# paulmillr/noble-curves

Measured on NVIDIA H100. Metric: BLS12-381 G1 MSM points/sec at 2^20 scalars, higher is better.
Workload: dtype u32-limb integer (381-bit Fp, Montgomery)

## Files before the change

### noble-curves_b200/csrc/ec.cuh

```cuda
#pragma once
#include "curve_consts.cuh"
#include "field.cuh"
#include "inv_divsteps.cuh"
#include "fp2.cuh"

namespace nmsm {

#if defined(__CUDACC__)
template <class F, bool FULLWARP>
struct Par4 {
  static constexpr int WORDS = sizeof(F) / 4;
  __device__ static __forceinline__ F bcast(const F& z, int src) {
    F r;
    const uint32_t* s = reinterpret_cast<const uint32_t*>(&z);
    uint32_t* d = reinterpret_cast<uint32_t*>(&r);
    const unsigned qbase = FULLWARP ? 0u : (threadIdx.x & 28u);
    const unsigned qmask = FULLWARP ? 0xffffffffu : (0xFu << qbase);
#pragma unroll
    for (int k = 0; k < WORDS; k++) d[k] = __shfl_sync(qmask, s[k], qbase + src);
    return r;
  }
  __device__ static __forceinline__ F pick(int l, const F& a0, const F& a1, const F& a2, const F& a3) {
    F r;
    const uint32_t* p0 = reinterpret_cast<const uint32_t*>(&a0);
// ... 3 lines not shown
    uint32_t* d = reinterpret_cast<uint32_t*>(&r);
    const uint32_t m0 = 0u - (uint32_t)(l == 0), m1 = 0u - (uint32_t)(l == 1), m2 = 0u - (uint32_t)(l == 2),
                   m3 = 0u - (uint32_t)(l == 3);
#pragma unroll
    for (int k = 0; k < WORDS; k++) d[k] = (p0[k] & m0) | (p1[k] & m1) | (p2[k] & m2) | (p3[k] & m3);
    return r;
  }
  __device__ static __forceinline__ void mul4(F& r0, F& r1, F& r2, F& r3, const F& a0, const F& b0, const F& a1,
                                              const F& b1, const F& a2, const F& b2, const F& a3, const F& b3) {
    const int l = threadIdx.x & 3;
    F x = pick(l, a0, a1, a2, a3), y = pick(l, b0, b1, b2, b3);
    F z = x * y;
    r0 = bcast(z, 0);
    r1 = bcast(z, 1);
    r2 = bcast(z, 2);
    r3 = bcast(z, 3);
  }
};
#endif

template <class F>
struct SwXyzz {
  using Field = F;
  static constexpr int COORD_WORDS = F::LIMBS;
  static constexpr int IN_WORDS = 2 * F::LIMBS;
  static constexpr int AFF_WORDS = 2 * F::LIMBS;
  static constexpr int ACC_WORDS = 4 * F::LIMBS;
  static constexpr int COST_MADD = 10, COST_ADD = 14, COST_DBL = 9;
  static constexpr bool IS_EDWARDS = false;

  struct Affine {
    F x, y;
  };
  struct Acc {
    F X, Y, ZZ, ZZZ;
  };

  NMSM_HD static Acc identity() { return Acc{F::zero(), F::one(), F::zero(), F::zero()}; }
  NMSM_HD static bool is_identity(const Acc& p) { return p.ZZ.is_zero(); }
  NMSM_HD static bool affine_is_identity(const Affine& a) { return a.x.is_zero() && a.y.is_zero(); }
  NMSM_HD static Affine prepare(const uint32_t* xy) {
    return Affine{F::from_canonical(xy), F::from_canonical(xy + F::LIMBS)};
  }
  NMSM_HD static bool input_in_range(const uint32_t* xy) {
    return F::canonical_in_range(xy) && F::canonical_in_range(xy + F::LIMBS);
  }
  NMSM_HD static Affine neg(const Affine& a) { return Affine{a.x, -a.y}; }
  NMSM_HD static Affine cneg(const Affine& a, bool n) {
    F ny = -a.y;
    return Affine{a.x, n ? ny : a.y};
  }
  NMSM_HD static Acc from_affine(const Affine& a) {
    if (affine_is_identity(a)) return identity();
    return Acc{a.x, a.y, F::one(), F::one()};
  }
  NMSM_HD static Acc neg(const Acc& p) { return Acc{p.X, -p.Y, p.ZZ, p.ZZZ}; }

  NMSM_HD static Acc dbl_affine(const Affine& a) {
    F U = nmsm::dbl(a.y);
    F V = sqr(U);
    F W = U * V;
    F S = a.x * V;
    F xx = sqr(a.x);
    F M = nmsm::dbl(xx) + xx;
    F X3 = sqr(M) - nmsm::dbl(S);
    F Y3 = M * (S - X3) - W * a.y;
    return Acc{X3, Y3, V, W};
  }
  NMSM_HD static void dbl(Acc& p) {
    if (is_identity(p)) return;
    F U = nmsm::dbl(p.Y);
    F V = sqr(U);
    F W = U * V;
    F S = p.X * V;
    F xx = sqr(p.X);
    F M = nmsm::dbl(xx) + xx;
    F X3 = sqr(M) - nmsm::dbl(S);
    F Y3 = M * (S - X3) - W * p.Y;
    p.ZZ = V * p.ZZ;
    p.ZZZ = W * p.ZZZ;
    p.X = X3;
    p.Y = Y3;
  }
  NMSM_HD static void madd(Acc& p, const Affine& a) {
    if (affine_is_identity(a)) return;
    if (is_identity(p)) {
      p = Acc{a.x, a.y, F::one(), F::one()};
      return;
    }
    F U2 = a.x * p.ZZ;
    F S2 = a.y * p.ZZZ;
    F P = U2 - p.X;
    F R = S2 - p.Y;
    if (P.is_zero()) {
      if (R.is_zero())
        p = dbl_affine(a);
      else
        p = identity();
      return;
    }
    F PP = sqr(P);
    F PPP = P * PP;
    F Q = p.X * PP;
    F X3 = sqr(R) - PPP - nmsm::dbl(Q);
    F Y3 = R * (Q - X3) - p.Y * PPP;
    p.ZZ = p.ZZ * PP;
    p.ZZZ = p.ZZZ * PPP;
    p.X = X3;
    p.Y = Y3;
  }
  NMSM_HD static void add(Acc& p, const Acc& q) {
    if (is_identity(q)) return;
    if (is_identity(p)) {
      p = q;
      return;
    }
    F U1 = p.X * q.ZZ;
    F U2 = q.X * p.ZZ;
    F S1 = p.Y * q.ZZZ;
    F S2 = q.Y * p.ZZZ;
    F P = U2 - U1;
    F R = S2 - S1;
    if (P.is_zero()) {
      if (R.is_zero())
        dbl(p);
      else
        p = identity();
      return;
    }
    F PP = sqr(P);
    F PPP = P * PP;
    F Q = U1 * PP;
    F X3 = sqr(R) - PPP - nmsm::dbl(Q);
    F Y3 = R * (Q - X3) - S1 * PPP;
    p.ZZ = p.ZZ * q.ZZ * PP;
    p.ZZZ = p.ZZZ * q.ZZZ * PPP;
    p.X = X3;
    p.Y = Y3;
  }
#if defined(__CUDACC__)
  template <bool FW>
  __device__ static void par_dbl(Acc& p) {
    if (is_identity(p)) return;
    using P4 = Par4<F, FW>;
    F U = nmsm::dbl(p.Y);
    F V, A, t2, t3;
    P4::mul4(V, A, t2, t3, U, U, p.X, p.X, U, U, U, U);
    F M = nmsm::dbl(A) + A;
    F W, S, MM;
    P4::mul4(W, S, MM, t3, U, V, p.X, V, M, M, M, M);
    F X3 = MM - nmsm::dbl(S);
    F y0, y1, zz, zzz;
    P4::mul4(y0, y1, zz, zzz, M, S - X3, W, p.Y, V, p.ZZ, W, p.ZZZ);
    p.X = X3;
    p.Y = y0 - y1;
    p.ZZ = zz;
    p.ZZZ = zzz;
  }
  template <bool FW>
  __device__ static void par_add(Acc& p, const Acc& q) {
    if (is_identity(q)) return;
    if (is_identity(p)) {
      p = q;
      return;
    }
    using P4 = Par4<F, FW>;
    F U1, U2, S1, S2;
    P4::mul4(U1, U2, S1, S2, p.X, q.ZZ, q.X, p.ZZ, p.Y, q.ZZZ, q.Y, p.ZZZ);
    F P = U2 - U1;
    F R = S2 - S1;
    if (P.is_zero()) {
      if (R.is_zero())
        par_dbl<FW>(p);
      else
        p = identity();
      return;
    }
    F PP, RR, ZZ12, ZZZ12;
    P4::mul4(PP, RR, ZZ12, ZZZ12, P, P, R, R, p.ZZ, q.ZZ, p.ZZZ, q.ZZZ);
    F PPP, Q, ZZ3, t3;
    P4::mul4(PPP, Q, ZZ3, t3, P, PP, U1, PP, ZZ12, PP, P, PP);
    F X3 = RR - PPP - nmsm::dbl(Q);
    F y0, y1, ZZZ3;
    P4::mul4(y0, y1, ZZZ3, t3, R, Q - X3, S1, PPP, ZZZ12, PPP, R, R);
    p.X = X3;
    p.Y = y0 - y1;
    p.ZZ = ZZ3;
    p.ZZZ = ZZZ3;
  }
#endif
// ... 240 lines not shown
```

### noble-curves_b200/csrc/field.cuh

```cuda
#pragma once
#include "bigint.cuh"

namespace nmsm {

template <class C>
NMSM_HD void reduce_once(uint32_t* r, uint32_t top) {
  constexpr int N = C::N;
  uint32_t d[N];
  d[0] = sub_cc(r[0], C::P(0));
#pragma unroll
  for (int k = 1; k < N; k++) d[k] = subc_cc(r[k], C::P(k));
  uint32_t t = subc(top, 0);
  bool keep = (t >> 31) != 0;
#pragma unroll
  for (int k = 0; k < N; k++) r[k] = keep ? r[k] : d[k];
}

template <class C>
NMSM_HD void mont_mul(uint32_t* r, const uint32_t* a, const uint32_t* b) {
  constexpr int N = C::N;
  static_assert(N % 2 == 0, "even limb count expected");
  uint32_t E[2 * N + 2], O[2 * N + 2];
#pragma unroll
  for (int k = 0; k < 2 * N + 2; k++) {
// ... 247 lines not shown
  NMSM_HD friend Fp operator*(const Fp& a, const Fp& b) {
#if defined(__CUDA_ARCH__) && defined(NMSM_MUL_NOINLINE)
    return mul_call<C>(a, b);
#else
    Fp r;
    mont_mul<C>(r.v, a.v, b.v);
    return r;
#endif
  }
  NMSM_HD friend Fp operator+(const Fp& a, const Fp& b) {
    Fp r;
    r.v[0] = add_cc(a.v[0], b.v[0]);
#pragma unroll
    for (int k = 1; k < N; k++) r.v[k] = addc_cc(a.v[k], b.v[k]);
    uint32_t top = addc(0, 0);
    reduce_once<C>(r.v, top);
    return r;
  }
  NMSM_HD friend Fp operator-(const Fp& a, const Fp& b) {
    Fp r;
    r.v[0] = sub_cc(a.v[0], b.v[0]);
#pragma unroll
    for (int k = 1; k < N; k++) r.v[k] = subc_cc(a.v[k], b.v[k]);
    uint32_t mask = subc(0, 0);
    r.v[0] = add_cc(r.v[0], C::P(0) & mask);
#pragma unroll
    for (int k = 1; k < N; k++) r.v[k] = addc_cc(r.v[k], C::P(k) & mask);
    return r;
  }
  NMSM_HD Fp operator-() const { return zero() - *this; }

  NMSM_HD static Fp from_canonical(const uint32_t* x) {
    Fp a, r2;
#pragma unroll
    for (int k = 0; k < N; k++) {
      a.v[k] = x[k];
      r2.v[k] = C::R2(k);
    }
    return a * r2;
  }
  NMSM_HD void to_canonical(uint32_t* x) const {
    Fp o;
#pragma unroll
    for (int k = 0; k < N; k++) o.v[k] = (k == 0) ? 1u : 0u;
    Fp r = (*this) * o;
#pragma unroll
    for (int k = 0; k < N; k++) x[k] = r.v[k];
  }
  NMSM_HD static bool canonical_in_range(const uint32_t* x) {
    uint32_t t = sub_cc(x[0], C::P(0));
#pragma unroll
    for (int k = 1; k < N; k++) t = subc_cc(x[k], C::P(k));
    (void)t;
    return subc(0, 0) != 0;
  }
};

#if defined(__CUDACC__)
template <class C>
__device__ __noinline__ Fp<C> mul_call(Fp<C> a, Fp<C> b) {
  Fp<C> r;
  mont_mul<C>(r.v, a.v, b.v);
  return r;
}
template <class C>
__device__ __noinline__ Fp<C> sqr_call(Fp<C> a) {
  Fp<C> r;
  mont_sqr<C>(r.v, a.v);
  return r;
}
#endif

template <class C>
NMSM_HD Fp<C> sqr(const Fp<C>& a) {
#if defined(__CUDA_ARCH__) && defined(NMSM_MUL_NOINLINE)
  return sqr_call<C>(a);
#else
  Fp<C> r;
  mont_sqr<C>(r.v, a.v);
  return r;
#endif
}
template <class C>
NMSM_HD Fp<C> dbl(const Fp<C>& a) {
  return a + a;
}

template <class C>
NMSM_HD Fp<C> inv_xgcd(const Fp<C>& a) {
  constexpr int N = C::N;
  if (a.is_zero()) return a;
  uint32_t u[N], v[N], x1[N], x2[N];
#pragma unroll
  for (int k = 0; k < N; k++) {
    u[k] = a.v[k];
    v[k] = C::P(k);
    x1[k] = (k == 0) ? 1u : 0u;
    x2[k] = 0u;
  }
  auto is_one = [](const uint32_t* x) {
    uint32_t t = x[0] ^ 1u;
#pragma unroll
    for (int k = 1; k < N; k++) t |= x[k];
    return t == 0;
  };
  auto halve = [](uint32_t* x, uint32_t top) {
#pragma unroll
    for (int k = 0; k < N - 1; k++) x[k] = (x[k] >> 1) | (x[k + 1] << 31);
    x[N - 1] = (x[N - 1] >> 1) | (top << 31);
  };
  auto halve_mod = [&](uint32_t* x) {
    uint32_t top = 0;
    if (x[0] & 1u) {
      x[0] = add_cc(x[0], C::P(0));
#pragma unroll
      for (int k = 1; k < N; k++) x[k] = addc_cc(x[k], C::P(k));
      top = addc(0, 0);
    }
    halve(x, top);
  };
  auto geq = [](const uint32_t* x, const uint32_t* y) {
    uint32_t t = sub_cc(x[0], y[0]);
#pragma unroll
    for (int k = 1; k < N; k++) t = subc_cc(x[k], y[k]);
    (void)t;
    return subc(0, 0) == 0;
  };
  auto sub_plain = [](uint32_t* x, const uint32_t* y) {
    x[0] = sub_cc(x[0], y[0]);
#pragma unroll
    for (int k = 1; k < N; k++) x[k] = subc_cc(x[k], y[k]);
  };
  auto sub_mod = [](uint32_t* x, const uint32_t* y) {
    x[0] = sub_cc(x[0], y[0]);
#pragma unroll
    for (int k = 1; k < N; k++) x[k] = subc_cc(x[k], y[k]);
    uint32_t mask = subc(0, 0);
    x[0] = add_cc(x[0], C::P(0) & mask);
#pragma unroll
    for (int k = 1; k < N; k++) x[k] = addc_cc(x[k], C::P(k) & mask);
  };
  while (!is_one(u) && !is_one(v)) {
    while (!(u[0] & 1u)) {
      halve(u, 0);
      halve_mod(x1);
    }
    while (!(v[0] & 1u)) {
      halve(v, 0);
      halve_mod(x2);
    }
    if (geq(u, v)) {
      sub_plain(u, v);
      sub_mod(x1, x2);
    } else {
      sub_plain(v, u);
      sub_mod(x2, x1);
    }
  }
  Fp<C> r, r2;
  const bool pick_u = is_one(u);
#pragma unroll
  for (int k = 0; k < N; k++) {
    r.v[k] = pick_u ? x1[k] : x2[k];
    r2.v[k] = C::R2(k);
  }
  return (r * r2) * r2;
// ... 4 lines not shown
```

### noble-curves_b200/csrc/msm.cuh

```cuda
#pragma once
#include <cuda_runtime.h>
#include <stdint.h>

#include "msm_body.cuh"
#include "validate.cuh"

namespace nmsm {

template <class Cv>
__global__ void k_prepare(const uint32_t* __restrict__ pts, uint32_t n, uint32_t* __restrict__ aff,
                          unsigned int* err) {
  uint32_t i = blockIdx.x * blockDim.x + threadIdx.x;
  if (i < n) prepare_body<Cv>(i, n, pts, aff, err);
}

template <class Cv, bool SCATTER>
__global__ void k_digits(const uint32_t* __restrict__ scalars, uint32_t n, MsmPlan plan,
                         unsigned int* __restrict__ counts_or_cursor, uint32_t* __restrict__ sorted,
                         unsigned int* err) {
  uint32_t i = blockIdx.x * blockDim.x + threadIdx.x;
  if (i < n) digits_body<Cv, SCATTER>(i, n, scalars, plan, counts_or_cursor, sorted, err);
}

static constexpr int SCAN_THREADS = 256;
// ... 10 lines not shown
  return t;
}

static __global__ void __launch_bounds__(SCAN_THREADS)
k_scan_tiles(const unsigned int* __restrict__ counts, uint32_t G, uint32_t* __restrict__ tile_sums) {
  __shared__ uint32_t sh[SCAN_THREADS / 32];
  const uint32_t base = blockIdx.x * SCAN_TILE + threadIdx.x * SCAN_PER_THREAD;
  uint32_t v = 0;
#pragma unroll
  for (int k = 0; k < SCAN_PER_THREAD; k++)
    if (base + k < G) v += counts[base + k];
  uint32_t t = block_sum_256(v, sh);
  if (threadIdx.x == 0) tile_sums[blockIdx.x] = t;
}

static __global__ void __launch_bounds__(SCAN_THREADS)
k_scan_apply(const unsigned int* __restrict__ counts, uint32_t G, const uint32_t* __restrict__ tile_sums,
             uint32_t* __restrict__ offsets, unsigned int* __restrict__ cursor) {
  __shared__ uint32_t sh[SCAN_THREADS / 32];
  __shared__ uint32_t warp_tot[SCAN_THREADS / 32];
  uint32_t pre = 0;
  for (uint32_t k = threadIdx.x; k < blockIdx.x; k += SCAN_THREADS) pre += tile_sums[k];
  const uint32_t tile_prefix = block_sum_256(pre, sh);
  const uint32_t base = blockIdx.x * SCAN_TILE + threadIdx.x * SCAN_PER_THREAD;
  uint32_t c[SCAN_PER_THREAD];
  uint32_t mine = 0;
#pragma unroll
  for (int k = 0; k < SCAN_PER_THREAD; k++) {
    c[k] = (base + k < G) ? counts[base + k] : 0;
    mine += c[k];
  }
  const uint32_t lane = threadIdx.x & 31, warp = threadIdx.x >> 5;
  uint32_t inc = mine;
  for (int d = 1; d < 32; d <<= 1) {
    uint32_t o = __shfl_up_sync(0xffffffffu, inc, d);
    if (lane >= (uint32_t)d) inc += o;
  }
  if (lane == 31) warp_tot[warp] = inc;
  __syncthreads();
  uint32_t wpre = 0;
  for (uint32_t q = 0; q < warp; q++) wpre += warp_tot[q];
  uint32_t run = tile_prefix + wpre + inc - mine;
#pragma unroll
  for (int k = 0; k < SCAN_PER_THREAD; k++) {
    if (base + k < G) {
      offsets[base + k] = run;
      cursor[base + k] = run;
    }
    run += c[k];
  }
  if (base < G && base + SCAN_PER_THREAD >= G) offsets[G] = run;
}

template <class F>
__device__ __forceinline__ F shfl_field(const F& a, int src_lane) {
  F r;
  const uint32_t* s = reinterpret_cast<const uint32_t*>(&a);
  uint32_t* d = reinterpret_cast<uint32_t*>(&r);
#pragma unroll
  for (int k = 0; k < (int)(sizeof(F) / 4); k++) d[k] = __shfl_sync(0xffffffffu, s[k], src_lane);
  return r;
}
template <class F>
__device__ __noinline__ F warp_batch_inverse(const F& z) {
  const int lane = threadIdx.x & 31;
  F pre = z, suf = z;
  for (int d = 1; d < 32; d <<= 1) {
    F a = shfl_field(pre, lane >= d ? lane - d : lane);
    F b = shfl_field(suf, lane + d < 32 ? lane + d : lane);
    if (lane >= d) pre = pre * a;
    if (lane + d < 32) suf = suf * b;
  }
  F r = inv(shfl_field(pre, 31));
  F left = shfl_field(pre, lane > 0 ? lane - 1 : 0);
  F right = shfl_field(suf, lane < 31 ? lane + 1 : 31);
  if (lane > 0) r = r * left;
  if (lane < 31) r = r * right;
  return r;
}

#ifndef NMSM_PAIRED
#define NMSM_PAIRED 0
#endif
#ifndef NMSM_ACC_MINBLOCKS_WIDE
#define NMSM_ACC_MINBLOCKS_WIDE 2
#endif
#ifndef NMSM_ACC_WIDE_BYTES
#define NMSM_ACC_WIDE_BYTES 257
#endif
#ifndef NMSM_ACC_MINBLOCKS
#define NMSM_ACC_MINBLOCKS 4
#endif
template <class Cv>
__global__ void __launch_bounds__(128, (sizeof(typename Cv::G::Acc) >= NMSM_ACC_WIDE_BYTES ? NMSM_ACC_MINBLOCKS_WIDE : NMSM_ACC_MINBLOCKS))
k_accumulate(const uint32_t* __restrict__ aff, const uint32_t* __restrict__ sorted,
             const uint32_t* __restrict__ offsets, MsmPlan plan, uint32_t w0, uint32_t* __restrict__ buckets,
             uint32_t* __restrict__ heads, uint32_t* __restrict__ tails) {
  const uint32_t gid = blockIdx.x * blockDim.x + threadIdx.x;
  const uint32_t w = w0 + gid / plan.TPW, t = gid % plan.TPW;
#if NMSM_PAIRED
  if constexpr (!Cv::G::IS_EDWARDS) {
    using F = typename Cv::G::Field;
    F suf[MAX_PAIRS];
    int npairs;
    const F run = accumulate_pairs_pass1<Cv>(w, t, aff, sorted, offsets, plan, suf, npairs);
    const F inv_all = warp_batch_inverse(run);
    accumulate_pairs_pass2<Cv>(w, t, aff, sorted, offsets, plan, suf, npairs, inv_all, buckets, heads, tails);
    return;
  }
#endif
  accumulate_body<Cv>(w, t, aff, sorted, offsets, plan, buckets, heads, tails);
}

template <class G>
__device__ __forceinline__ typename G::Acc shfl_down_acc(const typename G::Acc& a, int delta) {
  typename G::Acc r;
  const uint32_t* s = reinterpret_cast<const uint32_t*>(&a);
  uint32_t* d = reinterpret_cast<uint32_t*>(&r);
#pragma unroll
  for (int k = 0; k < G::ACC_WORDS; k++) d[k] = __shfl_down_sync(0xffffffffu, s[k], delta);
  return r;
}

template <class Cv>
__global__ void __launch_bounds__(128)
k_stitch_tiles(const uint32_t* __restrict__ offsets, MsmPlan plan, uint32_t span, uint32_t j0, uint32_t j1,
               const uint32_t* __restrict__ in, uint32_t* __restrict__ out) {
  using G = typename Cv::G;
  const uint32_t j = j0 + ((blockIdx.x * blockDim.x + threadIdx.x) >> 5), lane = threadIdx.x & 31;
  if (j >= j1) return;
  if (!tile_is_uniform(offsets, plan, (uint64_t)j * span, span)) return;
  typename G::Acc acc = load_acc<G>(in + ((size_t)j * STITCH_FAN + lane) * G::ACC_WORDS);
  for (int d = 16; d >= 1; d >>= 1) {
    typename G::Acc o = shfl_down_acc<G>(acc, d);
    nl_add<G>(acc, o);
  }
  if (lane == 0) save_acc<G>(out + (size_t)j * G::ACC_WORDS, acc);
}

static constexpr int REDUCE1_THREADS = 128;
#if defined(__CUDACC__)
template <class G>
struct QuadOps {
  __device__ static void add(typename G::Acc& p, const typename G::Acc& q) { G::template par_add<false>(p, q); }
  __device__ static void dbl(typename G::Acc& p) { G::template par_dbl<false>(p); }
  __device__ static void madd(typename G::Acc& p, const typename G::Affine& q) { G::template par_add<false>(p, G::from_affine(q)); }
};
#endif
template <class Cv, bool QUAD>
__global__ void __launch_bounds__(REDUCE1_THREADS)
k_reduce1(const uint32_t* __restrict__ offsets, const uint32_t* __restrict__ buckets,
          const uint32_t* __restrict__ heads, const uint32_t* __restrict__ tails,
          const uint32_t* __restrict__ tile1, const uint32_t* __restrict__ tile2, MsmPlan plan, uint32_t id0,
          uint32_t id1, uint32_t* __restrict__ sums, uint32_t* __restrict__ wsums) {
  using G = typename Cv::G;
  const uint32_t gt = blockIdx.x * blockDim.x + threadIdx.x;
  const uint32_t id = id0 + (QUAD ? gt >> 2 : gt);
  if (id >= id1) return;
  if (QUAD) reduce1_body<Cv, QuadOps<G>>(id, offsets, buckets, heads, tails, tile1, tile2, plan, sums, wsums);
  else reduce1_body<Cv, SerialOps<G>>(id, offsets, buckets, heads, tails, tile1, tile2, plan, sums, wsums);
}

template <class Cv>
__global__ void __launch_bounds__(128)
k_bucket_finalize(const uint32_t* __restrict__ offsets, uint32_t* __restrict__ buckets, const uint32_t* __restrict__ heads,
                  const uint32_t* __restrict__ tails, const uint32_t* __restrict__ tile1, const uint32_t* __restrict__ tile2,
                  MsmPlan plan, uint32_t g0, uint32_t g1) {
  const uint32_t g = g0 + blockIdx.x * blockDim.x + threadIdx.x;
  if (g < g1) bucket_finalize_body<Cv>(g, offsets, buckets, heads, tails, tile1, tile2, plan);
}
template <class Cv>
__global__ void __launch_bounds__(128)
k_bucket_fold(uint32_t* __restrict__ own, const uint32_t* __restrict__ recv, int npeers, size_t stride_words, uint32_t B) {
  const uint32_t b = (blockIdx.x * blockDim.x + threadIdx.x) >> 2;
  if (b < B) bucket_fold_body<Cv, QuadOps<typename Cv::G>>(b, own, recv, npeers, stride_words);
}
template <class Cv>
// ... 293 lines not shown
```

### noble-curves_b200/csrc/msm_body.cuh

```cuda
#pragma once
#include <math.h>
#include <stdint.h>
#include <stdlib.h>

#include "ec.cuh"

#if defined(__CUDACC__)
#define NMSM_NL __host__ __device__ __noinline__
#else
#define NMSM_NL inline
#endif

namespace nmsm {

static constexpr int MAX_WINDOW_BITS = 16;
static constexpr int MAX_TABLE_BITS = 22;
static constexpr int SCALAR_WORDS = 8;

struct MsmPlan {
  int c;
  int W;
  int B;
  int G;
  int L;
  int K;
  int chunks;
  int D;
  uint32_t stride;
  int wb, r;
  uint32_t TPW;
};
NMSM_HD int plan_seg_len(double entries, int sm_count) {
  const double wave = (double)sm_count * 4.0 * 128.0;
  const double waves = ceil(entries / (64.0 * wave));
  int L = (int)ceil(entries / ((waves < 1.0 ? 1.0 : waves) * wave));
  return L < 4 ? 4 : (L > 64 ? 64 : L);
}
static constexpr uint32_t SEG_ALIGN = 1024;
NMSM_HD uint32_t plan_tpw(uint64_t max_window_entries, int L) {
  const uint64_t t = (max_window_entries + (uint32_t)L - 1) / (uint32_t)L;
  return (uint32_t)((t + SEG_ALIGN - 1) / SEG_ALIGN * SEG_ALIGN);
}
NMSM_HD int digit_width(const MsmPlan& p, int w) { return p.wb + (w < p.r ? 1 : 0); }
NMSM_HD int digit_offset(const MsmPlan& p, int w) { return w * p.wb + (w < p.r ? w : p.r); }

template <class Cv>
constexpr int glv_bits() {
  if constexpr (Cv::GLV) return Cv::Glv::BITS;
  else return Cv::Fn::BITS;
}
template <class Cv>
constexpr int split_of() { return Cv::GLV_KIND == 3 ? 4 : (Cv::GLV ? 2 : 1); }

template <class Cv>
inline MsmPlan make_plan(uint64_t n, int forced_c, int sm_count, uint64_t n_local = 0, int min_c = 2) {
  using G = typename Cv::G;
  using F = typename G::Field;
  const int bits = glv_bits<Cv>();
  const double terms = (double)n * split_of<Cv>();
  const double limb_ratio = (double)(F::LIMBS / F::BASE_MULS == 12 ? 1.0 : (8.0 * 8.0) / (12.0 * 12.0));
  const double fscale = limb_ratio * F::BASE_MULS;
  const double t_madd = 0.352e-6 * fscale * G::COST_MADD / 10.0;
  const double t_add_tp = 0.93e-6 * fscale * G::COST_ADD / 14.0;
  const double t_add_lat = 0.030 * fscale * G::COST_ADD / 14.0;
  const double t_dbl_par = 0.0062 * fscale;
  const int K = 8;
  auto seg_len = [&](double entries) { return plan_seg_len(entries, sm_count); };
  int best_c = min_c;
  double best = 1e300;
  for (int c = min_c; c <= MAX_WINDOW_BITS; c++) {
    const int W = (bits + 1 + c - 1) / c;
    const double B = (double)(1u << (c - 1));
    const double entries = terms * W;
    const int L = seg_len(entries);
    const double parts_avg = 1.0 + (terms / B) / L;
    const int top_bits = bits + 1 - (W - 1) * c;
    const double per_bucket_top = terms / (double)(1u << (top_bits > 1 ? top_bits - 1 : 0));
    double parts_top = 1.0 + per_bucket_top / L;
    if (parts_top > 100.0) parts_top = 100.0 + per_bucket_top / L / 32.0;
    const double kk = B < K ? B : K;
    const double t_acc = entries * t_madd;
    const double t_r1a = W * B * (1.0 + parts_avg) * t_add_tp, t_r1b = kk * (1.0 + parts_top) * t_add_lat;
    const double cost = t_acc + (t_r1a > t_r1b ? t_r1a : t_r1b) + 0.75 * fscale + (double)(W - 1) * c * t_dbl_par;
    if (cost < best) {
      best = cost;
      best_c = c;
    }
  }
  int c = (forced_c >= 1 && forced_c <= MAX_WINDOW_BITS) ? forced_c : best_c;
  if (c < min_c) c = min_c;
  MsmPlan p;
  p.c = c;
  p.W = (bits + 1 + c - 1) / c;
  p.B = 1 << (c - 1);
  p.G = p.W * p.B;
  const double terms_local = n_local ? (double)n_local * split_of<Cv>() : terms;
  p.L = seg_len(terms_local * p.W);
  const uint64_t nbuckets = (uint64_t)p.W * (uint64_t)p.B;
  int Kc = nbuckets <= 65536u ? 2 : (nbuckets <= 131072u ? 4 : K);
#if !defined(__CUDA_ARCH__)
  if (const char* e = getenv("NMSM_L")) { int v = atoi(e); if (v >= 1 && v <= 1024) p.L = v; }
  if (const char* e = getenv("NMSM_K")) { int v = atoi(e); if (v >= 1 && (v & (v - 1)) == 0) Kc = v; }
#endif
  p.K = p.B < Kc ? p.B : Kc;
  p.chunks = p.B / p.K;
  p.D = p.W;
  p.stride = 0;
  p.wb = p.c;
  p.r = 0;
  p.TPW = plan_tpw((uint64_t)terms_local, p.L);
  return p;
}

NMSM_HD bool reduce1_quad_form(const MsmPlan& p) { return p.stride == 0 && (uint64_t)p.W * (uint64_t)p.B <= 65536u; }

template <class Cv>
inline void plan_one_wave_per_window(MsmPlan& p, uint64_t n_local, int sm_count) {
  const double terms_local = (double)(n_local ? n_local : 1) * split_of<Cv>();
  int L1 = (int)ceil(terms_local / ((double)sm_count * 4.0 * 128.0));
  p.L = L1 < 4 ? 4 : (L1 > 64 ? 64 : L1);
  p.TPW = plan_tpw((uint64_t)terms_local, p.L);
}

template <class Cv>
inline int table_digits(int c) { return (glv_bits<Cv>() + 1 + c - 1) / c; }
template <class Cv>
inline int canonical_table_bits(int c_req) {
  const int T = glv_bits<Cv>() + 1;
  int c = c_req;
  for (int it = 0; it < 8; it++) {
    const int D = (T + c - 1) / c;
    const int c2 = (T + D - 1) / D;
    if (c2 == c) break;
    c = c2;
  }
  return c;
}

static constexpr int TABLE_REDUCE_CHUNK = 8;

template <class Cv>
inline int choose_table_bits(uint64_t n_points, int sm_count, double mem_budget_bytes) {
  using G = typename Cv::G;
  using F = typename G::Field;
  const int T = glv_bits<Cv>() + 1;
  const double terms = (double)n_points * split_of<Cv>();
  const double limb_ratio = (double)(F::LIMBS / F::BASE_MULS == 12 ? 1.0 : (8.0 * 8.0) / (12.0 * 12.0));
  const double fscale = limb_ratio * F::BASE_MULS;
  const double t_madd = 0.352e-6 * fscale * G::COST_MADD / 10.0;
  const double t_add_tp = 0.93e-6 * fscale * G::COST_ADD / 14.0;
  const double t_add_lat = 0.006 * fscale * G::COST_ADD / 14.0;
  const double t_level = 0.2 * fscale;
  int best_c = 4;
  double best = 1e300;
  for (int c0 = 4; c0 <= MAX_TABLE_BITS; c0++) {
    const int c = canonical_table_bits<Cv>(c0);
    if (c != c0) continue;
    const int D = table_digits<Cv>(c);
    if ((double)D * terms * G::AFF_WORDS * 4.0 > mem_budget_bytes && c > 4) continue;
    const int wb = T / D, r = T % D;
    const double B = (double)(1u << (c - 1));
    const double entries = terms * D;
    const int L = plan_seg_len(entries, sm_count);
    const double load_low = r ? terms * ((double)(D - r) / (double)(1u << (wb - 1)) + (double)r / (double)(1u << wb))
                              : entries / B;
    const double parts_top = 1.0 + load_low / L;
    const double kk = B < TABLE_REDUCE_CHUNK ? B : TABLE_REDUCE_CHUNK;
    const double t_r1a = (entries / L + 2.0 * B) * t_add_tp, t_r1b = kk * (1.0 + parts_top) * t_add_lat;
    const double chunks = B / kk;
    const int levels = chunks <= 4096.0 ? 1 : (chunks <= 524288.0 ? 2 : 3);
    const double cost = entries * t_madd + (t_r1a > t_r1b ? t_r1a : t_r1b) + levels * t_level;
    if (cost < best) {
      best = cost;
      best_c = c;
    }
  }
  return best_c;
}

template <class Cv>
inline MsmPlan make_table_plan(uint64_t n_points, int c, int sm_count) {
  MsmPlan p;
  const int T = glv_bits<Cv>() + 1;
  const double terms = (double)n_points * split_of<Cv>();
  p.D = table_digits<Cv>(c);
  p.wb = T / p.D;
  p.r = T % p.D;
  p.c = p.wb + (p.r ? 1 : 0);
  p.W = 1;
  p.B = 1 << (p.c - 1);
  p.G = p.B;
  p.stride = (uint32_t)(n_points * split_of<Cv>());
  p.L = plan_seg_len(terms * p.D, sm_count);
  int Kc = TABLE_REDUCE_CHUNK;
#if !defined(__CUDA_ARCH__)
  if (const char* e = getenv("NMSM_TK")) { int v = atoi(e); if (v >= 1 && (v & (v - 1)) == 0) Kc = v; }
#endif
  p.K = p.B < Kc ? p.B : Kc;
  p.chunks = p.B / p.K;
  p.TPW = plan_tpw((uint64_t)terms * p.D, p.L);
  return p;
}

template <class Cv>
inline uint64_t plan_modmuls(const MsmPlan& p, uint64_t entries) {
  using G = typename Cv::G;
  using F = typename G::Field;
  uint64_t per = F::BASE_MULS;
  uint64_t m = entries * G::COST_MADD + (uint64_t)p.W * 2ull * p.B * G::COST_ADD +
               (uint64_t)(p.W - 1) * p.c * G::COST_DBL;
  return m * per;
}

template <int WORDS>
NMSM_HD void load_words(uint32_t* dst, const uint32_t* src) {
  static_assert(WORDS % 4 == 0, "rows are 16-byte multiples");
#if defined(__CUDA_ARCH__)
  const uint4* s4 = reinterpret_cast<const uint4*>(src);
#pragma unroll
  for (int k = 0; k < WORDS / 4; k++) {
    uint4 v = __ldg(s4 + k);
    dst[4 * k + 0] = v.x;
    dst[4 * k + 1] = v.y;
    dst[4 * k + 2] = v.z;
    dst[4 * k + 3] = v.w;
  }
#else
  for (int k = 0; k < WORDS; k++) dst[k] = src[k];
#endif
}
template <int WORDS>
NMSM_HD void load_words_rw(uint32_t* dst, const uint32_t* src) {
#if defined(__CUDA_ARCH__)
  const uint4* s4 = reinterpret_cast<const uint4*>(src);
#pragma unroll
  for (int k = 0; k < WORDS / 4; k++) {
    uint4 v = s4[k];
    dst[4 * k + 0] = v.x;
    dst[4 * k + 1] = v.y;
    dst[4 * k + 2] = v.z;
    dst[4 * k + 3] = v.w;
  }
#else
  for (int k = 0; k < WORDS; k++) dst[k] = src[k];
#endif
}
template <int WORDS>
NMSM_HD void store_words(uint32_t* dst, const uint32_t* src) {
#if defined(__CUDA_ARCH__)
  uint4* d4 = reinterpret_cast<uint4*>(dst);
#pragma unroll
  for (int k = 0; k < WORDS / 4; k++) d4[k] = make_uint4(src[4 * k], src[4 * k + 1], src[4 * k + 2], src[4 * k + 3]);
#else
  for (int k = 0; k < WORDS; k++) dst[k] = src[k];
#endif
}
NMSM_HD uint32_t atomic_add_u32(unsigned int* p, uint32_t v) {
#if defined(__CUDA_ARCH__)
  return atomicAdd(p, v);
#else
  uint32_t o = *p;
  *p += v;
  return o;
#endif
}
NMSM_HD void atomic_min_u32(unsigned int* p, uint32_t v) {
#if defined(__CUDA_ARCH__)
  atomicMin(p, v);
#else
  if (v < *p) *p = v;
#endif
}

template <class G>
NMSM_HD typename G::Acc load_acc(const uint32_t* src) {
  typename G::Acc a;
  load_words_rw<G::ACC_WORDS>(reinterpret_cast<uint32_t*>(&a), src);
  return a;
}
template <class G>
NMSM_HD void save_acc(uint32_t* dst, const typename G::Acc& a) {
  store_words<G::ACC_WORDS>(dst, reinterpret_cast<const uint32_t*>(&a));
}
template <class G>
NMSM_HD typename G::Affine load_aff(const uint32_t* src) {
  typename G::Affine a;
  load_words<G::AFF_WORDS>(reinterpret_cast<uint32_t*>(&a), src);
  return a;
}

template <class G>
NMSM_NL void nl_add(typename G::Acc& p, const typename G::Acc& q) { G::add(p, q); }
template <class G>
NMSM_NL void nl_dbl(typename G::Acc& p) { G::dbl(p); }
template <class G>
NMSM_NL void nl_madd(typename G::Acc& p, const typename G::Affine& a) { G::madd(p, a); }
template <class G>
NMSM_NL void nl_to_affine(const typename G::Acc& p, uint32_t* xy, uint32_t* inf) {
  G::to_affine_canonical(p, xy, inf);
}

template <class G>
struct SerialOps {
  NMSM_HD static void add(typename G::Acc& p, const typename G::Acc& q) { nl_add<G>(p, q); }
  NMSM_HD static void dbl(typename G::Acc& p) { nl_dbl<G>(p); }
  NMSM_HD static void madd(typename G::Acc& p, const typename G::Affine& q) { nl_madd<G>(p, q); }
};
template <class G>
struct InlineOps {
  NMSM_HD static void add(typename G::Acc& p, const typename G::Acc& q) { G::add(p, q); }
  NMSM_HD static void dbl(typename G::Acc& p) { G::dbl(p); }
};

NMSM_HD uint32_t scalar_bits(const uint32_t* s, int off, int c, int nwords = SCALAR_WORDS) {
  int w = off >> 5, sh = off & 31;
  if (w >= nwords) return 0;
  uint64_t lo = s[w];
  uint64_t hi = (w + 1 < nwords) ? s[w + 1] : 0;
  uint64_t v = (lo | (hi << 32)) >> sh;
  return (uint32_t)v & ((1u << c) - 1u);
}

template <class Fn>
NMSM_HD bool scalar_in_range(const uint32_t* s) {
  uint32_t t = sub_cc(s[0], Fn::ORDER(0));
#pragma unroll
  for (int k = 1; k < SCALAR_WORDS; k++) t = subc_cc(s[k], Fn::ORDER(k));
  (void)t;
  return subc(0, 0) != 0;
// ... 346 lines not shown
  return true;
}

template <bool SCATTER>
NMSM_HD void emit_digits(const uint32_t* m, int nwords, uint32_t index, uint32_t flip, const MsmPlan& plan,
                         unsigned int* counts_or_cursor, uint32_t* sorted) {
  uint32_t carry = 0;
  for (int w = 0; w < plan.D; w++) {
    const int width = digit_width(plan, w);
    const uint32_t half = 1u << (width - 1);
    uint32_t v = scalar_bits(m, digit_offset(plan, w), width, nwords) + carry;
    carry = 0;
    uint32_t neg = flip;
    if (v > half) {
      v = (1u << width) - v;
      neg ^= 1u;
      carry = 1;
    }
    if (v != 0) {
      const uint32_t g = (plan.stride ? 0u : (uint32_t)w * (uint32_t)plan.B) + (v - 1);
      if (SCATTER) {
        uint32_t pos = atomic_add_u32(&counts_or_cursor[g], 1u);
        sorted[pos] = (index + (uint32_t)w * plan.stride) | (neg << 31);
      } else {
        atomic_add_u32(&counts_or_cursor[g], 1u);
      }
    }
  }
}

template <class Cv, bool SCATTER>
NMSM_HD void digits_body(uint32_t i, uint32_t n, const uint32_t* scalars, const MsmPlan& plan,
                         unsigned int* counts_or_cursor, uint32_t* sorted, unsigned int* err) {
  uint32_t s[SCALAR_WORDS];
  load_words<SCALAR_WORDS>(s, scalars + (size_t)i * SCALAR_WORDS);
  if (!scalar_in_range<typename Cv::Fn>(s)) {
    if (!SCATTER) atomic_min_u32(&err[1], i);
    return;
  }
  if constexpr (Cv::GLV_KIND == 1) {
    uint32_t m1[4], m2[4];
    bool neg1, neg2;
    glv_split<typename Cv::Glv>(s, m1, neg1, m2, neg2);
    emit_digits<SCATTER>(m1, 4, i, neg1 ? 1u : 0u, plan, counts_or_cursor, sorted);
    emit_digits<SCATTER>(m2, 4, n + i, neg2 ? 1u : 0u, plan, counts_or_cursor, sorted);
  } else if constexpr (Cv::GLV_KIND == 2) {
    uint32_t m1[5], m2[5];
    bool neg1, neg2;
    glv_split_lattice<typename Cv::Glv>(s, m1, neg1, m2, neg2);
    emit_digits<SCATTER>(m1, 5, i, neg1 ? 1u : 0u, plan, counts_or_cursor, sorted);
    emit_digits<SCATTER>(m2, 5, n + i, neg2 ? 1u : 0u, plan, counts_or_cursor, sorted);
  } else if constexpr (Cv::GLV_KIND == 3) {
    uint64_t mag[4];
    bool neg[4];
    gls_split<typename Cv::Glv>(s, mag, neg);
    for (int j = 0; j < 4; j++) {
      const uint32_t m[2] = {(uint32_t)mag[j], (uint32_t)(mag[j] >> 32)};
      emit_digits<SCATTER>(m, 2, (uint32_t)j * n + i, (neg[j] ? 1u : 0u) ^ (uint32_t)(j & 1), plan, counts_or_cursor, sorted);
    }
  } else {
    emit_digits<SCATTER>(s, SCALAR_WORDS, i, 0u, plan, counts_or_cursor, sorted);
  }
}

template <class Cv>
NMSM_HD void accumulate_body(uint32_t w, uint32_t t, const uint32_t* aff, const uint32_t* sorted, const uint32_t* offsets,
                             const MsmPlan& plan, uint32_t* buckets, uint32_t* heads, uint32_t* tails) {
  using G = typename Cv::G;
  const uint32_t g_lo = w * (uint32_t)plan.B, g_hi = g_lo + (uint32_t)plan.B;
  const uint32_t base = offsets[g_lo], T = offsets[g_hi];
  const uint64_t seg64 = (uint64_t)base + (uint64_t)t * (uint32_t)plan.L;
  if (seg64 >= T) return;
  const uint32_t seg = (uint32_t)seg64;
  const uint32_t end = (T - seg > (uint32_t)plan.L) ? seg + plan.L : T;
  const size_t sid = (size_t)w * plan.TPW + t;
  uint32_t lo = g_lo, hi = g_hi;
  while (hi - lo > 1) {
    uint32_t mid = (lo + hi) >> 1;
    if (offsets[mid] <= seg) lo = mid; else hi = mid;
  }
  uint32_t g = lo;
  uint32_t bstart = offsets[g], bend = offsets[g + 1];
  typename G::Acc acc = G::identity();
  for (uint32_t pos = seg; pos < end; pos++) {
    if (pos == bend) {
      if (bstart >= seg) save_acc<G>(buckets + (size_t)g * G::ACC_WORDS, acc);
      else save_acc<G>(heads + sid * G::ACC_WORDS, acc);
      acc = G::identity();
      do { g++; } while (offsets[g + 1] <= pos);
      bstart = offsets[g];
      bend = offsets[g + 1];
    }
    uint32_t e = sorted[pos];
    typename G::Affine a = load_aff<G>(aff + (size_t)(e & 0x7fffffffu) * G::AFF_WORDS);
    a = G::cneg(a, (e >> 31) != 0);
    G::madd(acc, a);
  }
  const bool head_open = bstart < seg;
  const bool tail_open = bend > end;
  if (!head_open && !tail_open) save_acc<G>(buckets + (size_t)g * G::ACC_WORDS, acc);
  else if (head_open) save_acc<G>(heads + sid * G::ACC_WORDS, acc);
  else save_acc<G>(tails + sid * G::ACC_WORDS, acc);
}

static constexpr int MAX_PAIRS = 32;

template <class F>
NMSM_HD bool pair_usable(const F& x1, const F& x2) {
  return !x1.is_zero() && !x2.is_zero() && x1 != x2;
}

template <class Cv>
NMSM_HD typename Cv::G::Field accumulate_pairs_pass1(uint32_t w, uint32_t t, const uint32_t* aff, const uint32_t* sorted,
                                                     const uint32_t* offsets, const MsmPlan& plan,
                                                     typename Cv::G::Field* suf, int& npairs) {
  using G = typename Cv::G;
  using F = typename G::Field;
  npairs = 0;
  F run = F::one();
  const uint32_t g_lo = w * (uint32_t)plan.B, g_hi = g_lo + (uint32_t)plan.B;
  const uint32_t base = offsets[g_lo], T = offsets[g_hi];
  const uint64_t seg64 = (uint64_t)base + (uint64_t)t * (uint32_t)plan.L;
  if (seg64 >= T) return run;
  const uint32_t seg = (uint32_t)seg64;
  const uint32_t end = (T - seg > (uint32_t)plan.L) ? seg + plan.L : T;
  uint32_t lo = g_lo, hi = g_hi;
  while (hi - lo > 1) {
    uint32_t mid = (lo + hi) >> 1;
    if (offsets[mid] <= end - 1) lo = mid; else hi = mid;
  }
  uint32_t g = lo;
  uint32_t pos = end;
  while (pos > seg) {
    while (offsets[g] >= pos) g--;
    const uint32_t b0 = offsets[g];
    const uint32_t rs = b0 > seg ? b0 : seg;
    if (pos - rs >= 2) {
      long long p = (long long)pos - 2;
      if ((((uint32_t)p - b0) & 1u) != 0) p--;
      for (; p >= (long long)rs; p -= 2) {
        const uint32_t e1 = sorted[p], e2 = sorted[p + 1];
        F x1, x2;
        load_words<F::LIMBS>(reinterpret_cast<uint32_t*>(&x1), aff + (size_t)(e1 & 0x7fffffffu) * G::AFF_WORDS);
        load_words<F::LIMBS>(reinterpret_cast<uint32_t*>(&x2), aff + (size_t)(e2 & 0x7fffffffu) * G::AFF_WORDS);
        if (pair_usable(x1, x2)) {
          suf[npairs++] = run;
          run = run * (x2 - x1);
        }
      }
    }
    pos = rs;
  }
  return run;
}

template <class Cv>
NMSM_HD void accumulate_pairs_pass2(uint32_t w, uint32_t t, const uint32_t* aff, const uint32_t* sorted, const uint32_t* offsets,
                                    const MsmPlan& plan, const typename Cv::G::Field* suf, int npairs,
                                    typename Cv::G::Field inv_all, uint32_t* buckets, uint32_t* heads, uint32_t* tails) {
  using G = typename Cv::G;
  using F = typename G::Field;
  const uint32_t g_lo = w * (uint32_t)plan.B, g_hi = g_lo + (uint32_t)plan.B;
  const uint32_t base = offsets[g_lo], T = offsets[g_hi];
  const uint64_t seg64 = (uint64_t)base + (uint64_t)t * (uint32_t)plan.L;
  if (seg64 >= T) return;
  const uint32_t seg = (uint32_t)seg64;
  const uint32_t end = (T - seg > (uint32_t)plan.L) ? seg + plan.L : T;
  const size_t sid = (size_t)w * plan.TPW + t;
  uint32_t lo = g_lo, hi = g_hi;
  while (hi - lo > 1) {
    uint32_t mid = (lo + hi) >> 1;
    if (offsets[mid] <= seg) lo = mid; else hi = mid;
  }
  uint32_t g = lo;
  uint32_t bstart = offsets[g], bend = offsets[g + 1];
  typename G::Acc acc = G::identity();
  int k = 0;
  for (uint32_t pos = seg; pos < end;) {
    if (pos == bend) {
// ... 407 lines not shown
```

Baseline: 106.5 million.

## Double-buffer affine point loads via cp.async and inline madd products for G1

For accumulator types of 192 bytes (BLS12-381 G1 XYZZ), the bucket accumulation loop now prefetches the next affine point into a shared-memory double buffer with cp.async, overlapping the gather latency with the current mixed addition. It also forces the field multiplies and squares in madd to be inlined rather than going through possibly non-inlined calls, and sets launch bounds to 3 blocks per SM for this size. Segment-length planning is updated to use the per-type blocks-per-SM value. This aims to hide global memory latency and call overhead, at the cost of shared memory usage, register pressure and code size.

```diff
diff --git a/noble-curves_b200/csrc/ec.cuh b/noble-curves_b200/csrc/ec.cuh
--- a/noble-curves_b200/csrc/ec.cuh
+++ b/noble-curves_b200/csrc/ec.cuh
@@ -109,14 +109,23 @@
     p.X = X3;
     p.Y = Y3;
   }
+  template <bool INL = false>
   NMSM_HD static void madd(Acc& p, const Affine& a) {
+    auto mul = [](const F& x, const F& y) -> F {
+      if constexpr (INL) return mul_inline(x, y);
+      else return x * y;
+    };
+    auto sq = [](const F& x) -> F {
+      if constexpr (INL) return sqr_inline(x);
+      else return sqr(x);
+    };
     if (affine_is_identity(a)) return;
     if (is_identity(p)) {
       p = Acc{a.x, a.y, F::one(), F::one()};
       return;
     }
-    F U2 = a.x * p.ZZ;
-    F S2 = a.y * p.ZZZ;
+    F U2 = mul(a.x, p.ZZ);
+    F S2 = mul(a.y, p.ZZZ);
     F P = U2 - p.X;
     F R = S2 - p.Y;
     if (P.is_zero()) {
@@ -126,13 +135,13 @@
         p = identity();
       return;
     }
-    F PP = sqr(P);
-    F PPP = P * PP;
-    F Q = p.X * PP;
-    F X3 = sqr(R) - PPP - nmsm::dbl(Q);
-    F Y3 = R * (Q - X3) - p.Y * PPP;
-    p.ZZ = p.ZZ * PP;
-    p.ZZZ = p.ZZZ * PPP;
+    F PP = sq(P);
+    F PPP = mul(P, PP);
+    F Q = mul(p.X, PP);
+    F X3 = sq(R) - PPP - nmsm::dbl(Q);
+    F Y3 = mul(R, Q - X3) - mul(p.Y, PPP);
+    p.ZZ = mul(p.ZZ, PP);
+    p.ZZZ = mul(p.ZZZ, PPP);
     p.X = X3;
     p.Y = Y3;
   }
diff --git a/noble-curves_b200/csrc/field.cuh b/noble-curves_b200/csrc/field.cuh
--- a/noble-curves_b200/csrc/field.cuh
+++ b/noble-curves_b200/csrc/field.cuh
@@ -353,6 +353,18 @@
 #endif
 }
 template <class C>
+NMSM_HD Fp<C> mul_inline(const Fp<C>& a, const Fp<C>& b) {
+  Fp<C> r;
+  mont_mul<C>(r.v, a.v, b.v);
+  return r;
+}
+template <class C>
+NMSM_HD Fp<C> sqr_inline(const Fp<C>& a) {
+  Fp<C> r;
+  mont_sqr<C>(r.v, a.v);
+  return r;
+}
+template <class C>
 NMSM_HD Fp<C> dbl(const Fp<C>& a) {
   return a + a;
 }
diff --git a/noble-curves_b200/csrc/msm.cuh b/noble-curves_b200/csrc/msm.cuh
--- a/noble-curves_b200/csrc/msm.cuh
+++ b/noble-curves_b200/csrc/msm.cuh
@@ -116,17 +116,8 @@
 #ifndef NMSM_PAIRED
 #define NMSM_PAIRED 0
 #endif
-#ifndef NMSM_ACC_MINBLOCKS_WIDE
-#define NMSM_ACC_MINBLOCKS_WIDE 2
-#endif
-#ifndef NMSM_ACC_WIDE_BYTES
-#define NMSM_ACC_WIDE_BYTES 257
-#endif
-#ifndef NMSM_ACC_MINBLOCKS
-#define NMSM_ACC_MINBLOCKS 4
-#endif
-template <class Cv>
-__global__ void __launch_bounds__(128, (sizeof(typename Cv::G::Acc) >= NMSM_ACC_WIDE_BYTES ? NMSM_ACC_MINBLOCKS_WIDE : NMSM_ACC_MINBLOCKS))
+template <class Cv>
+__global__ void __launch_bounds__(128, acc_blocks_per_sm<typename Cv::G>())
 k_accumulate(const uint32_t* __restrict__ aff, const uint32_t* __restrict__ sorted,
              const uint32_t* __restrict__ offsets, MsmPlan plan, uint32_t w0, uint32_t* __restrict__ buckets,
              uint32_t* __restrict__ heads, uint32_t* __restrict__ tails) {
diff --git a/noble-curves_b200/csrc/msm_body.cuh b/noble-curves_b200/csrc/msm_body.cuh
--- a/noble-curves_b200/csrc/msm_body.cuh
+++ b/noble-curves_b200/csrc/msm_body.cuh
@@ -30,8 +30,16 @@
   int wb, r;
   uint32_t TPW;
 };
-NMSM_HD int plan_seg_len(double entries, int sm_count) {
-  const double wave = (double)sm_count * 4.0 * 128.0;
+template <class G>
+NMSM_HD constexpr int acc_blocks_per_sm() {
+  return sizeof(typename G::Acc) == 192 ? 3 : (sizeof(typename G::Acc) > 256 ? 2 : 4);
+}
+template <class G>
+NMSM_HD constexpr bool acc_inline_products() {
+  return acc_blocks_per_sm<G>() == 3;
+}
+NMSM_HD int plan_seg_len(double entries, int sm_count, int blocks_per_sm) {
+  const double wave = (double)sm_count * blocks_per_sm * 128.0;
   const double waves = ceil(entries / (64.0 * wave));
   int L = (int)ceil(entries / ((waves < 1.0 ? 1.0 : waves) * wave));
   return L < 4 ? 4 : (L > 64 ? 64 : L);
@@ -65,7 +73,7 @@
   const double t_add_lat = 0.030 * fscale * G::COST_ADD / 14.0;
   const double t_dbl_par = 0.0062 * fscale;
   const int K = 8;
-  auto seg_len = [&](double entries) { return plan_seg_len(entries, sm_count); };
+  auto seg_len = [&](double entries) { return plan_seg_len(entries, sm_count, acc_blocks_per_sm<G>()); };
   int best_c = min_c;
   double best = 1e300;
   for (int c = min_c; c <= MAX_WINDOW_BITS; c++) {
@@ -117,7 +125,7 @@
 template <class Cv>
 inline void plan_one_wave_per_window(MsmPlan& p, uint64_t n_local, int sm_count) {
   const double terms_local = (double)(n_local ? n_local : 1) * split_of<Cv>();
-  int L1 = (int)ceil(terms_local / ((double)sm_count * 4.0 * 128.0));
+  int L1 = (int)ceil(terms_local / ((double)sm_count * acc_blocks_per_sm<typename Cv::G>() * 128.0));
   p.L = L1 < 4 ? 4 : (L1 > 64 ? 64 : L1);
   p.TPW = plan_tpw((uint64_t)terms_local, p.L);
 }
@@ -161,7 +169,7 @@
     const int wb = T / D, r = T % D;
     const double B = (double)(1u << (c - 1));
     const double entries = terms * D;
-    const int L = plan_seg_len(entries, sm_count);
+    const int L = plan_seg_len(entries, sm_count, acc_blocks_per_sm<G>());
     const double load_low = r ? terms * ((double)(D - r) / (double)(1u << (wb - 1)) + (double)r / (double)(1u << wb))
                               : entries / B;
     const double parts_top = 1.0 + load_low / L;
@@ -191,7 +199,7 @@
   p.B = 1 << (p.c - 1);
   p.G = p.B;
   p.stride = (uint32_t)(n_points * split_of<Cv>());
-  p.L = plan_seg_len(terms * p.D, sm_count);
+  p.L = plan_seg_len(terms * p.D, sm_count, acc_blocks_per_sm<typename Cv::G>());
   int Kc = TABLE_REDUCE_CHUNK;
 #if !defined(__CUDA_ARCH__)
   if (const char* e = getenv("NMSM_TK")) { int v = atoi(e); if (v >= 1 && (v & (v - 1)) == 0) Kc = v; }
@@ -245,6 +253,18 @@
   for (int k = 0; k < WORDS; k++) dst[k] = src[k];
 #endif
 }
+#if defined(__CUDA_ARCH__)
+template <int WORDS>
+__device__ __forceinline__ void load_words_async(uint4 (*dst)[128], const uint32_t* src) {
+  static_assert(WORDS % 4 == 0, "rows are 16-byte multiples");
+#pragma unroll
+  for (int k = 0; k < WORDS / 4; k++) {
+    const uint32_t d = (uint32_t)__cvta_generic_to_shared(&dst[k][threadIdx.x]);
+    asm volatile("cp.async.cg.shared.global [%0], [%1], 16;" ::"r"(d), "l"(src + 4 * k) : "memory");
+  }
+  asm volatile("cp.async.commit_group;" ::: "memory");
+}
+#endif
 template <int WORDS>
 NMSM_HD void store_words(uint32_t* dst, const uint32_t* src) {
 #if defined(__CUDA_ARCH__)
@@ -757,19 +777,52 @@
   uint32_t g = lo;
   uint32_t bstart = offsets[g], bend = offsets[g + 1];
   typename G::Acc acc = G::identity();
-  for (uint32_t pos = seg; pos < end; pos++) {
-    if (pos == bend) {
-      if (bstart >= seg) save_acc<G>(buckets + (size_t)g * G::ACC_WORDS, acc);
-      else save_acc<G>(heads + sid * G::ACC_WORDS, acc);
-      acc = G::identity();
-      do { g++; } while (offsets[g + 1] <= pos);
-      bstart = offsets[g];
-      bend = offsets[g + 1];
-    }
-    uint32_t e = sorted[pos];
-    typename G::Affine a = load_aff<G>(aff + (size_t)(e & 0x7fffffffu) * G::AFF_WORDS);
-    a = G::cneg(a, (e >> 31) != 0);
-    G::madd(acc, a);
+  auto next_bucket = [&](uint32_t pos) {
+    if (bstart >= seg) save_acc<G>(buckets + (size_t)g * G::ACC_WORDS, acc);
+    else save_acc<G>(heads + sid * G::ACC_WORDS, acc);
+    acc = G::identity();
+    do { g++; } while (offsets[g + 1] <= pos);
+    bstart = offsets[g];
+    bend = offsets[g + 1];
+  };
+#if defined(__CUDA_ARCH__)
+  if constexpr (acc_inline_products<G>()) {
+    constexpr int Q = G::AFF_WORDS / 4;
+    __shared__ uint4 next_pts[2][Q][128];
+    uint32_t e = sorted[seg], e_next = seg + 1 < end ? sorted[seg + 1] : 0u;
+    load_words_async<G::AFF_WORDS>(next_pts[0], aff + (size_t)(e & 0x7fffffffu) * G::AFF_WORDS);
+    for (uint32_t pos = seg, slot = 0; pos < end; pos++, slot ^= 1u) {
+      if (pos == bend) next_bucket(pos);
+      const uint32_t e_after = pos + 2 < end ? sorted[pos + 2] : 0u;
+      if (pos + 1 < end) load_words_async<G::AFF_WORDS>(next_pts[slot ^ 1u], aff + (size_t)(e_next & 0x7fffffffu) * G::AFF_WORDS);
+      else asm volatile("cp.async.commit_group;" ::: "memory");
+      asm volatile("cp.async.wait_group 1;" ::: "memory");
+      typename G::Affine a;
+      uint32_t* aw = reinterpret_cast<uint32_t*>(&a);
+#pragma unroll
+      for (int k = 0; k < Q; k++) {
+        const uint4 v = next_pts[slot][k][threadIdx.x];
+        aw[4 * k] = v.x;
+        aw[4 * k + 1] = v.y;
+        aw[4 * k + 2] = v.z;
+        aw[4 * k + 3] = v.w;
+      }
+      a = G::cneg(a, (e >> 31) != 0);
+      G::template madd<true>(acc, a);
+      e = e_next;
+      e_next = e_after;
+    }
+  } else
+#endif
+  {
+    for (uint32_t pos = seg; pos < end; pos++) {
+      if (pos == bend) next_bucket(pos);
+      uint32_t e = sorted[pos];
+      typename G::Affine a = load_aff<G>(aff + (size_t)(e & 0x7fffffffu) * G::AFF_WORDS);
+      a = G::cneg(a, (e >> 31) != 0);
+      if constexpr (acc_inline_products<G>()) G::template madd<true>(acc, a);
+      else G::madd(acc, a);
+    }
   }
   const bool head_open = bstart < seg;
   const bool tail_open = bend > end;
```

Result: faster. 110.3 million (median of 6 runs) (+3.6%).
